# COPT-Public/LoRADS

Measured on AMD Instinct MI355X. Metric: ADMM iters/sec (+ inner CG-iters/sec), single-block n=20000 r=40, higher is better.
Workload: dtype f64

## Files before the change

### include/lorads_hip.h

```cpp
#ifndef LORADS_HIP_H
#define LORADS_HIP_H

#include <stdint.h>

#ifdef __cplusplus
extern "C" {
#endif

typedef struct lorads_hip_ctx lorads_hip_ctx;

typedef struct {
    int32_t n;
    int32_t rank;
    int32_t nrow;
    const int32_t *row_idx;
    const int32_t *a_ptr;
    const int32_t *a_row;
    const int32_t *a_col;
    const double *a_val;
    int32_t c_nnz;
    const int32_t *c_row;
    const int32_t *c_col;
    const double *c_val;
    int32_t is_lp;
// ... 59 lines not shown

int lorads_hip_triangle_cuts(lorads_hip_ctx *ctx, int32_t src, int32_t blk, double min_violation, int32_t max_cuts, int64_t *count,
                             int32_t *p, int32_t *q, int32_t *s, int8_t *cls, double *viol, int32_t *kept, int32_t *passes);

int lorads_hip_alm_to_admm(lorads_hip_ctx *ctx);
int lorads_hip_average_uv_to_v(lorads_hip_ctx *ctx);
int lorads_hip_scale_obj(lorads_hip_ctx *ctx, double s);
int lorads_hip_resize_rank(lorads_hip_ctx *ctx, const int32_t *new_rank);
int lorads_hip_set_mat(lorads_hip_ctx *ctx, int32_t which, int32_t blk, const double *colmajor);
int lorads_hip_get_mat(lorads_hip_ctx *ctx, int32_t which, int32_t blk, double *colmajor);
int lorads_hip_set_vec(lorads_hip_ctx *ctx, int32_t which, const double *v);
int lorads_hip_get_vec(lorads_hip_ctx *ctx, int32_t which, double *v);
int lorads_hip_set_allreduce(lorads_hip_ctx *ctx, lorads_hip_allreduce_fn fn, void *user);
void *lorads_hip_stream(lorads_hip_ctx *ctx);
int lorads_hip_set_allreduce_stream_ordered(lorads_hip_ctx *ctx, int32_t on);
int lorads_hip_set_separable(lorads_hip_ctx *ctx, int32_t on);
typedef int (*lorads_hip_scalar_exchange_fn)(void *user, double *vals, int32_t n);
int lorads_hip_set_scalar_exchange(lorads_hip_ctx *ctx, lorads_hip_scalar_exchange_fn fn, void *user);
int lorads_hip_selfcheck_allreduce(lorads_hip_ctx *ctx);

int lorads_hip_sync(lorads_hip_ctx *ctx);
int lorads_hip_spec_front_stats(lorads_hip_ctx *ctx, int64_t out[4]);

#ifdef __cplusplus
}
#endif
#endif
```

### lorads_amd/csrc/hip/graph.inc

```
struct MutSnap {
    InitArgs pend_init; Guard pend_init_g;
    Deferred pend_chk; Guard pend_chk_g;
    lorads_hip_ctx::PendDir pend_dir;
    lorads_hip_ctx::PendSegChk pend_segchk;
    bool pend_dual, pend_dual_virtual, virt_refresh, avg_folded, final_pending, stage_clean, merged_t_uv;
    EvalFinalArgs final_args;
    double *lambda, *lambda_alt;
    int ls_np, head;
    std::vector<unsigned char> blk;
    std::vector<const double *> wj_for;
};
struct GraphEntry {
    hipGraphExec_t exec = nullptr;
    MutSnap after;
    long d_matvec = 0;
    unsigned long long d_seq = 0;
};
struct GraphCache {
    std::map<std::vector<uint64_t>, GraphEntry> map;
    std::map<std::vector<uint64_t>, int> seen;
    long n_capture = 0, n_replay = 0;
};
void graph_cache_clear(lorads_hip_ctx *c) {
    if (!c->graphs) return;
    for (auto &kv : c->graphs->map)
        if (kv.second.exec) hipGraphExecDestroy(kv.second.exec);
    c->graphs->map.clear();
    c->graphs->seen.clear();
}
void graph_cache_free(lorads_hip_ctx *c) {
    graph_cache_clear(c);
    delete c->graphs;
    c->graphs = nullptr;
}
MutSnap snap_take(const lorads_hip_ctx *c) {
    MutSnap s;
    s.pend_init = c->pend_init; s.pend_init_g = c->pend_init_g; s.pend_chk = c->pend_chk; s.pend_chk_g = c->pend_chk_g;
    s.pend_dir = c->pend_dir; s.pend_segchk = c->pend_segchk;
    s.pend_dual = c->pend_dual; s.pend_dual_virtual = c->pend_dual_virtual; s.virt_refresh = c->virt_refresh; s.avg_folded = c->avg_folded;
// ... 62 lines not shown
int set_step_params(lorads_hip_ctx *c, double rho, double tol, int maxit) {
    const double v[4] = {rho, tol, c->pend_dual_rho, (double)maxit};
    const int mask = step_params_mask(c, v);
    if (!mask) return 0;
    hipLaunchKernelGGL(k_set_par, dim3(1), dim3(1), 0, c->stream, c->par, v[0], v[1], v[2], v[3], mask);
    for (int k = 0; k < 4; ++k)
        if ((mask >> k) & 1) { c->par_h[k] = v[k]; c->par_valid |= 1 << k; }
    return 0;
}

template <class F>
int graph_step(lorads_hip_ctx *c, std::vector<uint64_t> &key, F &&enqueue) {
    const MutSnap before = snap_take(c);
    if (!snap_quiet(before)) return enqueue();
    if (!c->graphs) c->graphs = new GraphCache();
    snap_key(c, before, key);
    auto it = c->graphs->map.find(key);
    if (it != c->graphs->map.end()) {
        const GraphEntry &e = it->second;
        HC(hipGraphLaunch(e.exec, c->stream));
        snap_put(c, e.after);
        c->n_matvec += e.d_matvec;
        c->pub_seq += e.d_seq;
        c->graphs->n_replay++;
        return 0;
    }
    if (c->graphs->seen.size() >= 4096) c->graphs->seen.clear();
    if (++c->graphs->seen[key] < 2) return enqueue();
    if (c->graphs->map.size() >= 256) graph_cache_clear(c);
    const long mv0 = c->n_matvec;
    const unsigned long long seq0 = c->pub_seq;
    auto give_up = [&](hipGraph_t g) {
        if (g) hipGraphDestroy(g);
        (void)hipGetLastError();
        c->opt_graph = false;
        snap_put(c, before);
        c->n_matvec = mv0;
        c->pub_seq = seq0;
        if (getenv("LORADS_HIP_VERBOSE")) fprintf(stderr, "lorads_hip: graph capture failed, launching step by step\n");
        return enqueue();
    };
    if (hipStreamBeginCapture(c->stream, hipStreamCaptureModeThreadLocal) != hipSuccess) return give_up(nullptr);
    const int rc = enqueue();
    hipGraph_t g = nullptr;
    const hipError_t e1 = hipStreamEndCapture(c->stream, &g);
    if (rc) {
        if (g) hipGraphDestroy(g);
        snap_put(c, before);
        c->n_matvec = mv0;
        c->pub_seq = seq0;
        return rc;
    }
    if (e1 != hipSuccess || !g) return give_up(g);
    GraphEntry ent;
    if (hipGraphInstantiate(&ent.exec, g, nullptr, nullptr, 0) != hipSuccess) return give_up(g);
    hipGraphDestroy(g);
    ent.after = snap_take(c);
    ent.d_matvec = c->n_matvec - mv0;
    ent.d_seq = c->pub_seq - seq0;
    HC(hipGraphLaunch(ent.exec, c->stream));
    c->graphs->map.emplace(key, std::move(ent));
    c->graphs->n_capture++;
    return 0;
}
```

### lorads_amd/csrc/hip/kernels.inc

```
template <int LG, bool V2, int NS>
struct Slice {
    static constexpr int W = V2 ? 2 : 1;
    __device__ static __forceinline__ void load(const double *__restrict__ row, int r, int lane, double (&v)[NS][W]) {
#pragma unroll
        for (int c = 0; c < NS; ++c) {
            const int j = (lane + c * LG) * W;
            const bool ok = j < r;
            const int jc = ok ? j : 0;
            if (V2) {
                const double2 t = *(const double2 *)(row + jc);
                v[c][0] = ok ? t.x : 0.0;
                v[c][W - 1] = ok ? t.y : 0.0;
            } else {
                const double t = row[jc];
                v[c][0] = ok ? t : 0.0;
            }
        }
    }
};

template <int LG, bool V2, int NS>
__device__ __forceinline__ double pair_dot(const double *__restrict__ X, const double *__restrict__ Y, int p, int q, int r,
                                           int lane) {
    constexpr int W = V2 ? 2 : 1;
// ... 97 lines not shown
                            : d.st ? !blocked_after(g, d, finish_deferred(d, dv, sh).done) : GATE_OPEN;
    if (live && act && lane64 == 0) {
        if (w_out) w_out[i] = s;
        if (vec) {
            const int gi = ra.b ? gi_pre : row_idx[i];
            if (mode == CV_SET) vec[gi] = s * scale;
            else if (mode == CV_ADD) vec[gi] += s * scale;
            else vec[gi] += s - cv[i];
        }
        if (cv) cv[i] = s;
    }
    if (ra.b) {
        double vd[2] = {0.0, 0.0};
        if (act && lane64 == 0) {
            const double bi = b_pre, t = bi - s * scale;
            vd[0] = t * t;
            vd[1] = bi * l_pre;
        }
        block_sum_n<2>(vd, sh);
        if (live && threadIdx.x == 0) { ra.part_v[blockIdx.x] = vd[0]; ra.part_d[blockIdx.x] = vd[1]; }
    }
}

template <int NS4, int NS>
__global__ __launch_bounds__(TPB) void k_eval_cw_obj(int nrow, int ell_w, const int *__restrict__ a_p, const double *__restrict__ a_val,
                                                     const int *__restrict__ a_q, const double *__restrict__ R, int r,
                                                     double *__restrict__ cv, const int *__restrict__ row_idx, double *__restrict__ vec,
                                                     ResArgs ra, int g_cw, int ne, const int *__restrict__ erow,
                                                     const int *__restrict__ ecol, const double *__restrict__ cval,
                                                     double *__restrict__ part_obj, Guard g, Deferred d) {
    __shared__ double sh[8];
    const Gate gt = gate_load(g);
    DefPriv dv{};
    if (d.st) dv = deferred_private(d);
    if ((int)blockIdx.x < g_cw) {
        constexpr int LG = 4, GR = 16;
        const int i = (blockIdx.x * TPB + threadIdx.x) >> 6, lane64 = threadIdx.x & 63;
        const int grp = lane64 / LG, lane = lane64 % LG;
        const bool act = i < nrow;
        const int ic = act ? i : 0;
        const int gi = row_idx[ic];
        const double bi = ra.b[gi], li = ra.lambda[gi];
        const int t0 = ic * ell_w, t1 = act ? t0 + ell_w : t0;
        double acc = 0.0;
        for (int t = t0 + grp; t < t1; t += GR) {
            const int p0 = a_p[t], q0 = a_q[t];
            const double c0 = a_val[t];
            acc += c0 * pair_dot<LG, true, NS4>(R, R, p0, q0, r, lane);
        }
        const double s = wave_sum(acc);
        const bool live = d.st ? !blocked_after(g, d, finish_deferred(d, dv, sh).done) : GATE_OPEN;
        if (live && act && lane64 == 0) { vec[gi] = s * 1.0; cv[i] = s; }
        double vd[2] = {0.0, 0.0};
        if (act && lane64 == 0) {
            const double t = bi - s * 1.0;
            vd[0] = t * t;
            vd[1] = bi * li;
        }
        block_sum_n<2>(vd, sh);
        if (live && threadIdx.x == 0) { ra.part_v[blockIdx.x] = vd[0]; ra.part_d[blockIdx.x] = vd[1]; }
        return;
    }
    constexpr int LG = 8, per = TPB / LG;
    const int bid = blockIdx.x - g_cw, nblk = gridDim.x - g_cw;
    const int lane = threadIdx.x % LG;
    double sacc = 0.0;
    for (int e = bid * per + threadIdx.x / LG; e < ne; e += nblk * per)
        sacc += pair_dot<LG, true, NS>(R, R, erow[e], ecol[e], r, lane) * cval[e];
    const bool live = d.st ? !blocked_after(g, d, finish_deferred(d, dv, sh).done) : GATE_OPEN;
    const double t = block_sum(sacc, sh);
    if (live && threadIdx.x == 0) part_obj[bid] = t;
}

__global__ void k_fill(size_t len, double v, double *__restrict__ y) {
    for (size_t i = (size_t)blockIdx.x * blockDim.x + threadIdx.x; i < len; i += (size_t)gridDim.x * blockDim.x) y[i] = v;
}

template <int LG, bool V2, int NS>
__device__ __forceinline__ void pair_dot_rd(const double *__restrict__ R, const double *__restrict__ D, int p, int q, int r,
                                            int lane, double &t1, double &t2) {
    constexpr int W = V2 ? 2 : 1;
    double rp[NS][W], rq[NS][W], dp[NS][W], dq[NS][W];
    Slice<LG, V2, NS>::load(R + (size_t)p * r, r, lane, rp);
    Slice<LG, V2, NS>::load(D + (size_t)q * r, r, lane, dq);
    Slice<LG, V2, NS>::load(R + (size_t)q * r, r, lane, rq);
    Slice<LG, V2, NS>::load(D + (size_t)p * r, r, lane, dp);
    double a1 = 0.0, a2 = 0.0, b1 = 0.0, b2 = 0.0;
#pragma unroll
    for (int c = 0; c < NS; ++c)
#pragma unroll
        for (int w = 0; w < W; ++w) {
            a1 += rp[c][w] * dq[c][w]; a2 += rq[c][w] * dp[c][w];
            b1 += dp[c][w] * dq[c][w]; b2 += dq[c][w] * dp[c][w];
        }
// ... 1761 lines not shown
    double acc = 0.0;
    for (int col = threadIdx.x; col < ncols; col += TPB) {
        double w = cobj[col];
        for (int t = ptr[col]; t < ptr[col + 1]; ++t) w += -lambda[grow[t]] * a[t];
        acc += fabs(w < 0.0 ? w : 0.0);
    }
    acc = block_sum(acc, sh);
    if (threadIdx.x == 0) *out = acc;
}

__global__ __launch_bounds__(TPB) void k_publish(const unsigned long long *__restrict__ src, int nwords, unsigned long long *dst,
                                                 unsigned long long *flag, unsigned long long *seq_dev) {
    const unsigned long long seq = *seq_dev + 1;
    for (int i = threadIdx.x; i < nwords; i += TPB) dst[i] = src[i];
    __threadfence_system();
    __syncthreads();
    if (threadIdx.x == 0) {
        *seq_dev = seq;
        __atomic_store_n(flag, seq, __ATOMIC_RELEASE);
        __threadfence_system();
    }
}

struct EvalFinalArgs {
    const double *part_v, *part_d, *obj_part;
    int np, nobj;
    double *out;
    Guard g;
};
__global__ __launch_bounds__(TPB) void k_publish_final(EvalFinalArgs fa, const unsigned long long *src, int nwords,
                                                       unsigned long long *dst, unsigned long long *flag, unsigned long long *seq_dev) {
    __shared__ double sh[12];
    const unsigned long long seq = *seq_dev + 1;
    constexpr int PW = 4;
    unsigned long long pre[PW];
#pragma unroll
    for (int k = 0; k < PW; ++k) {
        const int i = threadIdx.x + k * TPB;
        pre[k] = __builtin_nontemporal_load(src + (i < nwords ? i : 0));
    }
    const bool live = !blocked(fa.g);
    const double *const pp[3] = {fa.part_v, fa.part_d, fa.obj_part ? fa.obj_part : fa.part_v};
    const int nn[3] = {fa.np, fa.np, fa.obj_part ? fa.nobj : 0};
    double t3[3];
    private_partials_n<3>(pp, nn, t3);
    block_sum_n<3>(t3, sh);
    const double v = t3[0], d = t3[1], o = t3[2];
    if (live && threadIdx.x == 0) { fa.out[0] = v; fa.out[1] = d; if (fa.obj_part) fa.out[2] = o; }
    const bool own = (const double *)src == fa.out;
#pragma unroll
    for (int k = 0; k < PW; ++k) {
        const int i = threadIdx.x + k * TPB;
// ... 660 lines not shown
```

### lorads_amd/csrc/hip/lorads_hip.hip

```cpp
#include <hip/hip_runtime.h>

#include <fcntl.h>
#include <sys/file.h>
#include <unistd.h>

#include <algorithm>
#include <chrono>
#include <cmath>
#include <cstdint>
#include <cstdio>
#include <cstring>
#include <map>
#include <string>
#include <atomic>
#include <mutex>
#include <thread>
#include <tuple>
#include <type_traits>
#include <vector>

#include "lorads_hip.h"
#include "lorads_hip_dev.h"

namespace {
// ... 505 lines not shown
    long long n_dev_patterns = 0, n_checked_patterns = 0;
    bool opt_dense_cache = true;
    bool opt_front_diag = true;
    bool opt_eval_diag = true;
    bool opt_fold_avg = true;
    bool opt_tile_update = true;
    bool avg_folded = false;
    bool opt_front_lds = true;
    bool opt_front_cw = true;
    bool opt_fuse_cg0 = true;
    bool pend_dual_virtual = false;
    bool opt_spec_front = true;
    struct SpecFront {
        bool live = false;
        bool dual_seen = false;
        double rho = 0.0, rho_dual = 0.0;
        int wmode = 0;
        unsigned long long epoch = 0;
        CGState *reset = nullptr;
        int nreset = 0;
    } spec;
    unsigned long long spec_epoch = 0;
    long long n_spec_enq = 0, n_spec_adopt = 0, n_spec_discard = 0, n_spec_blocked = 0;
    bool opt_exact_refresh = false, opt_split_front = false;
    bool final_pending = false;
    EvalFinalArgs final_args;
    double *scal = nullptr;
    CGState *st = nullptr;
    CGState *st_shadow = nullptr;
    InitArgs pend_init{};
    Guard pend_init_g{};
    Deferred pend_chk{};
    Guard pend_chk_g{};
    bool opt_lazy_scalars = true;
    struct PendDir { int kind = 0; CGState *st = nullptr; double *r = nullptr, *p = nullptr; size_t len = 0; int gv = 0;
                     const double *rs_part = nullptr; int rs_np = 0; Guard g{}; bool seg = false; int half = 0;
                     const double *chk_part = nullptr; double chk_tol = 0; int chk_maxit = 0, chk_k = 0;
                     const double *rs_seg = nullptr; } pend_dir;
    struct PendSegChk { bool on = false; int half = 0, k = 0; const double *part = nullptr; double tol = 0; int maxit = 0;
                        bool ride_res = false; } pend_segchk;
    struct PendSegInit { bool on = false; int half = 0; double tol = 0; Guard front{}; const double *part_rr = nullptr, *part_b = nullptr; } pend_seginit;
    bool opt_seg_carry_init = true;
    lorads_hip_scalar_exchange_fn sx = nullptr;
    void *sx_user = nullptr;
    bool sx_pending = false;
    int sx_with_obj = 0;
// ... 81 lines not shown
        const size_t need = (std::max(rows_max, rows_all) + 3) / 4 + 1;
        if (need > ((size_t)1 << 27)) return fail_msg("cone dimension beyond 2^29 rows");
        c->maxpart = (int)std::max<size_t>((size_t)MINPART, (need + 255) & ~(size_t)255);
    }
    c->opt_pad_rank = env_on("LORADS_PAD_ODD_RANK");
    c->opt_dev_presolve = env_on("LORADS_DEV_PRESOLVE");
    c->opt_presolve_check = env_set("LORADS_PRESOLVE_CHECK");
    if (getenv("LORADS_DEV_PRESOLVE_MIN")) c->dev_presolve_min = (size_t)std::max(0ll, atoll(getenv("LORADS_DEV_PRESOLVE_MIN")));
    c->blk.resize(c->nb);
    for (int k = 0; k < c->nb; ++k)
        if (build_block(c, c->blk[k], prob->blocks[k])) return 1;
    if (build_merged(c, prob)) return 1;
    common_rank(c);
    refresh_merged(c);
    if (getenv("LORADS_HIP_VERBOSE"))
        fprintf(stderr, "lorads_hip: %d cone(s), merged view %s\n", c->nb, c->has_merged ? "on" : (c->merged_ok ? "off (ranks differ)" : "not applicable"));
    if (alloc_factors(c)) return 1;
    std::vector<double> hb(prob->b, prob->b + c->m);
    DevPool &M = c->mem;
    if (M.upload(&c->b, hb) || M.alloc(&c->lambda, (size_t)c->m) || M.alloc(&c->lambda_alt, (size_t)c->m) || M.alloc(&c->csum, (size_t)c->m + 2) ||
        M.alloc(&c->cstage, (size_t)c->m + 2 + MINPART) || M.alloc(&c->gram, 128) ||
        M.alloc(&c->q12, (size_t)2 * c->m + 2) || M.alloc(&c->part, (size_t)NSLOT * c->maxpart) ||
        M.alloc(&c->ctrl, 64 * sizeof(double) + sizeof(CGState) * (size_t)std::max(2 * c->nb, 1)) ||
        M.alloc(&c->ring_ab, (size_t)2 * c->L) || M.alloc(&c->par, 8) || M.alloc(&c->seq_dev, 2))
        return 1;
    HC(hipMemset(c->par, 0, sizeof(double) * 8));
    HC(hipMemset(c->seq_dev, 0, sizeof(unsigned long long) * 2));
    c->opt_graph = env_on("LORADS_GRAPH");
    c->opt_graph_batched = getenv("LORADS_GRAPH") && getenv("LORADS_GRAPH")[0] == '2';
    c->opt_graph_forced = getenv("LORADS_GRAPH") && (getenv("LORADS_GRAPH")[0] == '1' || getenv("LORADS_GRAPH")[0] == '2');
    if (M.alloc_pinned(&c->h_ctrl, 64 * sizeof(double) + sizeof(CGState) * (size_t)std::max(2 * c->nb, 1), hipHostMallocMapped) ||
        M.alloc_pinned(&c->h_flag, 64 / sizeof(*c->h_flag), hipHostMallocMapped))
        return 1;
    *c->h_flag = 0;
    HC(hipHostGetDevicePointer((void **)&c->h_ctrl_dev, c->h_ctrl, 0));
    HC(hipHostGetDevicePointer((void **)&c->h_flag_dev, c->h_flag, 0));
    c->use_publish = !getenv("LORADS_NO_PUBLISH");
    c->opt_lazy_scalars = env_on("LORADS_LAZY_SCALARS");
    c->opt_ar_fast = !env_set("LORADS_AR_PLAIN");
    c->opt_gram = env_on("LORADS_LBFGS_GRAM");
    c->opt_gram_single = getenv("LORADS_LBFGS_GRAM") && getenv("LORADS_LBFGS_GRAM")[0] == '2';
    c->opt_fuse_dir = env_on("LORADS_FUSE_DIR");
    c->opt_entry_bip = env_on("LORADS_ENTRY_BIP");
    c->opt_seg_carry = env_on("LORADS_SEG_CARRY");
    c->opt_seg_carry_init = env_on("LORADS_SEG_CARRY_INIT");
    c->opt_seg_virt = env_on("LORADS_SEG_VIRT");
    c->opt_seg_carry_dual = env_on("LORADS_SEG_CARRY_DUAL");
    c->opt_seg_carry_restart = env_on("LORADS_SEG_CARRY_RESTART");
    c->opt_cw_quad = env_on("LORADS_CW_QUAD");
    c->opt_front_cw = env_on("LORADS_FRONT_CW");
    c->opt_fuse_cg0 = env_on("LORADS_FUSE_CG0");
    c->opt_front_lds = env_on("LORADS_FRONT_LDS");
    c->opt_spec_front = env_on("LORADS_SPEC_FRONT");
    if (getenv("LORADS_SPEC_WINDOW")) c->spec_window = std::max(1, std::min(8, atoi(getenv("LORADS_SPEC_WINDOW"))));
    c->opt_fold_avg = env_on("LORADS_FOLD_AVG");
    c->opt_tile_update = env_on("LORADS_TILE_UPDATE");
    c->opt_eval_diag = env_on("LORADS_EVAL_DIAG");
    c->opt_front_diag = env_on("LORADS_FRONT_DIAG");
    c->opt_dense_cache = env_on("LORADS_DENSE_CACHE");
    c->opt_fuse_eval = env_on("LORADS_FUSE_EVAL");
    c->opt_dense_rem = env_on("LORADS_DENSE_REM");
    c->opt_exact_refresh = env_set("LORADS_EXACT_REFRESH");
    c->opt_split_front = env_set("LORADS_SPLIT_FRONT");
    c->scal = (double *)c->ctrl;
    c->st = (CGState *)(c->ctrl + 64 * sizeof(double));
    c->h_scal = (double *)c->h_ctrl;
    c->h_st = (CGState *)(c->h_ctrl + 64 * sizeof(double));
    HC(hipMemset(c->lambda, 0, sizeof(double) * (size_t)std::max(c->m, 1)));
    HC(hipMemset(c->csum, 0, sizeof(double) * (size_t)(c->m + 2)));
    HC(hipMemset(c->q12, 0, sizeof(double) * (size_t)(2 * c->m + 2)));
    HC(hipMemset(c->scal, 0, sizeof(double) * 64));
    HC(hipMemset(c->ring_ab, 0, sizeof(double) * (size_t)2 * c->L));
    HC(hipMemset(c->st, 0, sizeof(CGState) * (size_t)std::max(2 * c->nb, 1)));
    if (M.alloc(&c->st_shadow, (size_t)std::max(2 * c->nb, 1))) return 1;
    HC(hipMemset(c->st_shadow, 0, sizeof(CGState) * (size_t)std::max(2 * c->nb, 1)));
    c->persist = new PersistPlan();
// ... 860 lines not shown
    for (int i = 0; i < 16; ++i) ticks[i] = 0;
    if (c->persist && c->persist->valid && c->persist->stamps && c->persist_stamps) {
        HC(hipMemcpy(c->persist->h_stamps, c->persist->stamps, sizeof(unsigned long long) * 16, hipMemcpyDeviceToHost));
        for (int i = 0; i < 16; ++i) ticks[i] = c->persist->h_stamps[i];
        HC(hipMemset(c->persist->stamps, 0, sizeof(unsigned long long) * 16));
    }
    c->persist_stamps = enable != 0;
    return 0;
}

int lorads_hip_presolve_stats(lorads_hip_ctx *c, int64_t stats[2]) {
    spec_touch(c);
    stats[0] = c->n_dev_patterns;
    stats[1] = c->n_checked_patterns;
    return 0;
}

int lorads_hip_spec_front_stats(lorads_hip_ctx *c, int64_t out[4]) {
    if (!c || !out) return fail_msg("spec_front_stats: bad argument");
    out[0] = c->n_spec_enq; out[1] = c->n_spec_adopt; out[2] = c->n_spec_discard; out[3] = c->n_spec_blocked;
    return 0;
}

int lorads_hip_graph_stats(lorads_hip_ctx *c, int64_t stats[4]) {
    spec_touch(c);
    stats[0] = c->graphs ? c->graphs->n_capture : 0;
    stats[1] = c->graphs ? c->graphs->n_replay : 0;
    stats[2] = c->graphs ? (int64_t)c->graphs->map.size() : 0;
    stats[3] = graph_ok(c) ? 1 : 0;
    return 0;
}

int lorads_hip_algorithmic_bytes(lorads_hip_ctx *c, int32_t k, double *mv, double *cg) {
    spec_touch(c);
    if (k < 0 || k >= c->nb) return fail_msg("bad block");
    const Block &B = c->blk[k];
    const double F = 8.0 * (double)B.n * (double)B.rl;
    *mv = 4 * F + 32.0 * B.na + 16.0 * B.nrow;
    *cg = *mv + 9 * F;
    return 0;
}

}

#include "lanczos.inc"
#include "postsolve.inc"
// ... 6 lines not shown
```

### lorads_amd/csrc/hip/sweep.inc

```
void flush_pending(lorads_hip_ctx *c);
#define LAUNCH(kern, grid, ...)                                                                      \
    do {                                                                                             \
        const int grid__ = (int)(grid);                                                              \
        if (c->pend_init.st || c->pend_chk.st || c->pend_dir.kind || c->pend_dual || c->pend_dual_virtual || c->sep_pending || c->pend_seginit.on) flush_pending(c); \
        if (grid__ > 0) { ++c->n_launch; hipLaunchKernelGGL(kern, dim3(grid__), dim3(TPB), 0, c->stream, __VA_ARGS__); } \
    } while (0)
#define LAUNCH_LDS(kern, grid, lds, ...)                                                             \
    do {                                                                                             \
        const int grid__ = (int)(grid);                                                              \
        if (c->pend_init.st || c->pend_chk.st || c->pend_dir.kind || c->pend_dual || c->pend_dual_virtual || c->sep_pending || c->pend_seginit.on) flush_pending(c); \
        if (grid__ > 0) { ++c->n_launch; hipLaunchKernelGGL(kern, dim3(grid__), dim3(TPB), (size_t)(lds), c->stream, __VA_ARGS__); } \
    } while (0)
inline InitArgs take_init(lorads_hip_ctx *c) {
    const InitArgs ia = c->pend_init;
    c->pend_init = InitArgs{};
    return ia;
}
inline Deferred take_check(lorads_hip_ctx *c) {
    const Deferred d = c->pend_chk;
    c->pend_chk = Deferred{};
    return d;
}

struct Shape {
// ... 681 lines not shown
}
void refresh_after_solve(lorads_hip_ctx *c, Block &B, const int *need) {
    if (constr_by_recurrence(c, B) && B.t_uv_valid && B.nrow > 0) {
        const Deferred d = (c->pend_chk.st && need == &c->pend_chk.st->done && !c->pend_init.st) ? take_check(c) : Deferred{};
        LAUNCH(k_refresh_w, nblocks_for((size_t)B.nrow, TPB), B.nrow, (const double *)B.w_uv, B.cv, B.row_idx, c->csum,
               Guard{nullptr, need}, d, B.diag_only ? (const int *)B.diag_row : (const int *)nullptr,
               B.diag_only ? (const double *)B.diag_a : (const double *)nullptr);
        return;
    }
    constr_val(c, B, c->U + B.off, c->V + B.off, 1.0, B.cv, CV_DELTA, c->csum, Guard{nullptr, need});
}

void flush_final(lorads_hip_ctx *c);
int enqueue_publish(lorads_hip_ctx *c, size_t word0, size_t nwords) {
    if (c->sx_pending && (word0 > SX_WORD || word0 + nwords < SX_WORD + 4)) {
        const size_t w1 = std::max(word0 + nwords, (size_t)SX_WORD + 4);
        word0 = std::min(word0, (size_t)SX_WORD);
        nwords = w1 - word0;
    }
    const bool sep = c->sep_pending && !c->final_pending && c->sep_ex.n <= 4;
    if (sep) c->sep_pending = false;
    flush_pending(c);
    ++c->pub_seq;
    if (sep) {
        LAUNCH(k_publish_sep, 1, (const double *)c->sepbuf, c->scal, c->sep_with_obj, c->sep_ex.n, c->sep_ex.p[0], c->sep_ex.p[1], c->sep_ex.p[2],
               c->sep_ex.p[3], (const unsigned long long *)c->ctrl + word0, (int)nwords, (unsigned long long *)c->h_ctrl_dev + word0,
               c->h_flag_dev, c->seq_dev);
    } else if (c->final_pending) {
        LAUNCH(k_publish_final, 1, c->final_args, (const unsigned long long *)c->ctrl + word0, (int)nwords,
               (unsigned long long *)c->h_ctrl_dev + word0, c->h_flag_dev, c->seq_dev);
        c->final_pending = false;
    } else {
        LAUNCH(k_publish, 1, (const unsigned long long *)c->ctrl + word0, (int)nwords, (unsigned long long *)c->h_ctrl_dev + word0,
               c->h_flag_dev, c->seq_dev);
    }
    return 0;
}
int sx_exchange(lorads_hip_ctx *c) {
    if (!c->sx_pending) return 0;
    c->sx_pending = false;
    double v[4] = {c->h_scal[SX_WORD], c->h_scal[SX_WORD + 1], c->h_scal[SX_WORD + 2], c->h_scal[SX_WORD + 3]};
    if (!c->sx || c->sx(c->sx_user, v, 4)) return fail_msg("scalar exchange of separable shards failed (a rank that never arrived?)");
    c->n_sx++;
    c->h_scal[0] = v[0];
    c->h_scal[1] = v[1];
    if (c->sx_with_obj) c->h_scal[2] = v[2];
// ... 150 lines not shown
            }
        } else if (eval_follows && c->nb == 1 && stg == 0 && c->opt_lazy_scalars && constr_by_recurrence(c, B) && B.t_uv_valid &&
                   fused_front(c, B) && (B.use_cw || B.diag_only)) {
            c->virt_refresh = true;
        } else {
            if (stg == 2 * c->nb - 1 && (c->n_sweeps % 32) == 31) B.t_uv_valid = false;
            refresh_after_solve(c, B, &s.st->done);
        }
    }
}

int first_unfinished(lorads_hip_ctx *c, int first) {
    for (int stg = first; stg < 2 * c->nb; ++stg)
        if (c->h_st[stg].done == 0) return stg;
    return -1;
}

void flush_final(lorads_hip_ctx *c) {
    if (!c->final_pending) return;
    const EvalFinalArgs &fa = c->final_args;
    LAUNCH(k_eval_final, 1, fa.part_v, fa.part_d, fa.np, fa.out, fa.g, fa.obj_part, fa.nobj);
    c->final_pending = false;
}
int enqueue_eval(lorads_hip_ctx *c, int pair, const int *need, bool with_obj = true) {
    flush_final(c);
    const Guard g{nullptr, need};
    const bool vec = shard_vec(c);
    Block *Dc = solo(c);
    Block *D1 = (pair == LORADS_HIP_PAIR_UV && !vec && c->opt_eval_diag && Dc && Dc->diag_only && Dc->rc_w > 0 && Dc->nrow == c->m &&
                 c->m > 0 && Dc->w_uv && !c->avg_folded && !Dc->dense_c) ? Dc : nullptr;
    if (D1) {
    } else if (pair == LORADS_HIP_PAIR_UV && c->avg_folded && need) {
        c->avg_folded = false;
    } else if (pair == LORADS_HIP_PAIR_UV) {
        c->avg_folded = false;
        const Deferred d = (c->pend_chk.st && need == &c->pend_chk.st->done && !c->pend_init.st) ? take_check(c) : Deferred{};
        LAUNCH(k_average, grid1d(c->all_elem), c->all_elem, c->U, c->V, c->R, g, d);
    }
    Block *S1 = solo(c);
    if (S1 && (S1->nrow != c->m || S1->dense_c)) S1 = c->nb == 1 ? S1 : nullptr;
    const bool single = (S1 && S1->nrow == c->m) || (c->nb == 1 && c->blk[0].nrow == c->m);
    bool any_dense_a = false;
    for (auto &B0 : c->blk) any_dense_a = any_dense_a || B0.dense_a;
    const bool fold_res = single && !vec && c->m > 0 && !any_dense_a;
    c->ls_np = 0;
    double *dst = vec ? c->cstage : c->csum;
    std::vector<Block *> cones;
// ... 8 lines not shown
    }
    const bool ar_fast = vec && with_obj && c->ar_fast_all == 1 && cones.size() == 1;
    if ((!single || vec) && !(ar_fast && c->stage_clean)) LAUNCH(k_zero, grid1d((size_t)c->m), (size_t)c->m, dst, g);
    bool first_obj = true;
    const bool fold_obj = (c->nb == 1 || S1) && !vec;
    int nobj = 0, nres = 0;
    for (Block *bp : cones) {
        Block &B = *bp;
        if (D1 == &B && fold_res) {
            const Deferred d = (c->pend_chk.st && need == &c->pend_chk.st->done && !c->pend_init.st && !c->pend_dir.kind) ? take_check(c) : Deferred{};
            const Shape sh = shape_for(B.r);
            nres = nblocks_for((size_t)B.n, TPB / sh.lg);
            SHAPE_DISPATCH(sh, LAUNCH((k_eval_diag<LG_, V2_, NS_>), nres, B.n, (const double *)(c->U + B.off), (const double *)(c->V + B.off),
                                      c->R + B.off, B.r, B.rc_w, (const int *)B.rc_con, (const double *)B.diag_a,
                                      B.row_idx_identity ? (const int *)nullptr : (const int *)B.row_idx, B.cv, c->csum,
                                      (const double *)c->b, (const double *)c->lambda, part_slot(c, 8), part_slot(c, 9), g, d));
        } else if (fold_res && B.use_cw && with_obj && fold_obj && c->opt_fuse_eval && cw_quad(c, B) && B.nc > 0 && !B.dense_c &&
                   nblocks_for((size_t)B.nrow, TPB / 64) <= c->maxpart) {
            const Deferred d = (c->pend_chk.st && need == &c->pend_chk.st->done && !c->pend_init.st && !c->pend_dir.kind) ? take_check(c) : Deferred{};
            nres = nblocks_for((size_t)B.nrow, TPB / 64);
            nobj = std::min(nblocks_for((size_t)B.nc, TPB / 8), 2048);
            const int ns4 = (B.r + 7) / 8, ns = (B.r + 15) / 16;
            const ResArgs ra{c->b, c->lambda, part_slot(c, 8), part_slot(c, 9)};
#define EVF(A4, A8) LAUNCH((k_eval_cw_obj<A4, A8>), nres + nobj, B.nrow, B.ca_ell, (const int *)B.ca_row, (const double *)B.ca_val, (const int *)B.ca_col, \
                           (const double *)(c->R + B.off), B.r, B.cv, (const int *)B.row_idx, c->csum, ra, nres, B.nc, (const int *)B.c_row,           \
                           (const int *)B.c_col, (const double *)B.c_val, part_slot(c, 4), g, d)
            switch (ns4) {
            case 1: EVF(1, 1); break;
            case 2: EVF(2, 1); break;
            case 3: EVF(3, 2); break;
            case 4: EVF(4, 2); break;
            case 5: EVF(5, 3); break;
            default: EVF(6, 3); break;
            }
#undef EVF
            (void)ns;
            lp_col_values(c, B, c->R, c->R, g);
            continue;
        } else if (fold_res && B.use_cw && nblocks_for((size_t)B.nrow, TPB / 64) <= c->maxpart) {
            nres = cw(c, B, c->R + B.off, c->R + B.off, 1.0, (double *)nullptr, B.cv, (int)CV_SET, c->csum, g,
                      ResArgs{c->b, c->lambda, part_slot(c, 8), part_slot(c, 9)});
        } else if (fold_res) {
            pairdots(c, B.pa, c->R + B.off, c->R + B.off, B.r, B.T2, g);
            nres = std::min(nblocks_for((size_t)B.nrow, TPB / 8), 2048);
            LAUNCH(k_cv_res, nres, B.nrow, B.a_ptr, B.a_e, B.a_val, B.T2, B.cv, B.row_idx, c->csum, c->b, c->lambda, part_slot(c, 8),
                   part_slot(c, 9), g);
        } else {
            constr_val(c, B, c->R + B.off, c->R + B.off, 1.0, B.cv, (single && !vec) ? CV_SET : CV_ADD, dst, g);
        }
// ... 14 lines not shown
        nres = std::max(1, std::min(grid1d((size_t)c->m), 256));
        LAUNCH(k_commit_eval, nres, c->m, dst, c->csum, c->b, c->lambda, part_slot(c, 8), part_slot(c, 9), c->scal,
               ar_fast ? nobj : 0);
        c->stage_clean = ar_fast;
    } else if (!fold_res) {
        nres = std::min(grid1d((size_t)c->m), 1024);
        LAUNCH(k_eval_part, nres, c->m, c->b, c->csum, c->lambda, part_slot(c, 8), part_slot(c, 9), g);
    }
    const double *op = (fold_obj && nobj > 0) ? part_slot(c, 4) : (const double *)nullptr;
    if (c->ar && c->sep) {
        const SepExtra ex = c->sep_extra;
        c->sep_extra = SepExtra{};
        if (c->sx && ex.n == 0 && c->use_publish) {
            LAUNCH(k_sep_stage_local, 1, part_slot(c, 8), part_slot(c, 9), nres, op, nobj, (const double *)c->scal, g, with_obj ? 1 : 0, c->scal + SX_WORD);
            c->sx_pending = true; c->sx_with_obj = with_obj ? 1 : 0;
            return 0;
        }
        LAUNCH(k_sep_stage, 1, part_slot(c, 8), part_slot(c, 9), nres, op, nobj, (const double *)c->scal, g, with_obj ? 1 : 0, c->sepbuf, ex);
        flush_pending(c);
        if (allreduce_dev(c, c->sepbuf, 4 + ex.n)) return 1;
        c->sep_pending = true; c->sep_with_obj = with_obj ? 1 : 0; c->sep_ex = ex;
        return 0;
    }
    if (c->use_publish) {
        c->final_args = EvalFinalArgs{part_slot(c, 8), part_slot(c, 9), op, nres, nobj, c->scal, g};
        c->final_pending = true;
    } else {
        LAUNCH(k_eval_final, 1, part_slot(c, 8), part_slot(c, 9), nres, c->scal, g, op, nobj);
    }
    return 0;
}

int read_scalars_at(lorads_hip_ctx *c, const double *dptr, int count, double *out) {
    flush_pending(c);
    flush_final(c);
    if (c->launch_err) { const char *e = c->launch_err; c->launch_err = nullptr; hipStreamSynchronize(c->stream); return fail_msg(e); }
    HC(hipMemcpyAsync(c->h_scal + 32, dptr, sizeof(double) * (size_t)count, hipMemcpyDeviceToHost, c->stream));
    HC(hipStreamSynchronize(c->stream));
    memcpy(out, c->h_scal + 32, sizeof(double) * (size_t)count);
    return 0;
}
int read_scalars(lorads_hip_ctx *c, int first, int count, double *out) {
    if (publish_and_wait(c, (size_t)first, (size_t)count)) return 1;
    memcpy(out, c->h_scal + first, sizeof(double) * (size_t)count);
    return 0;
}

// ... 233 lines not shown
        if (read_states(c)) return 1;
    }
    return 0;
}

bool persist_ready(lorads_hip_ctx *c, int maxit);
int run_sweep_persist(lorads_hip_ctx *c, double rho, double tol, int maxit, bool with_eval);
int run_sweep(lorads_hip_ctx *c, double rho, double tol, int maxit, bool with_eval) {
    if (persist_ready(c, maxit)) { spec_touch(c); return run_sweep_persist(c, rho, tol, maxit, with_eval); }
    persist_touch(c);
    if (c->has_merged && !getenv("LORADS_NO_BATCH")) { spec_touch(c); return run_sweep_batched(c, rho, tol, maxit, with_eval); }
    int first = 0, resume = -1;
    bool first_pass = true, any_missed = false;
    const bool graph = graph_this_step(c, rho, tol, maxit);
    if (graph && set_step_params(c, rho, tol, maxit)) return 1;
    ParMode pm(c, graph);
    if (graph || maxit < 1) spec_touch(c);
    const bool spec = with_eval && !graph && spec_front_ok(c);
    for (;;) {
        const bool eval_now = with_eval && (!c->ar || first_pass);
        auto enq = [&]() -> int {
            if (first_pass && 2 * c->nb - 1 > TPB) HC(hipMemsetAsync(c->st, 0, sizeof(CGState) * (size_t)(2 * c->nb), c->stream));
            enqueue_sweep(c, first, resume, rho, tol, maxit, with_eval);
            if (eval_now && enqueue_eval(c, LORADS_HIP_PAIR_UV, c->nb ? &c->st[2 * c->nb - 1].done : nullptr)) return 1;
            return c->use_publish ? enqueue_publish(c, 0, state_words(c)) : 0;
        };
        if (graph && first_pass) {
            std::vector<uint64_t> key{1, (uint64_t)with_eval, (uint64_t)maxit, (uint64_t)((c->n_sweeps % 32) == 31)};
            if (graph_step(c, key, enq)) return 1;
        } else if (enq()) return 1;
        if (spec && first_pass) spec_front_enqueue(c, rho);
        if (c->use_publish ? wait_publish(c) : read_states(c)) return 1;
        if (eval_now && c->ar) any_missed = c->h_scal[5] > 0.5;
        const int stg = first_unfinished(c, first);
        if (first_pass && c->spec.live && stg >= 0) { c->spec.live = false; ++c->n_spec_blocked; }
        first_pass = false;
        if (stg < 0) break;
        first = stg;
        resume = c->h_st[stg].iter;
        c->n_resume++;
        c->merged.t_uv_valid = false;
        for (auto &B : c->blk) { B.t_uv_valid = false; B.w0_ready = false; B.wj_for = nullptr; }
    }
    if (with_eval && c->ar && any_missed) {
        if (enqueue_eval(c, LORADS_HIP_PAIR_UV, nullptr)) return 1;
        if (read_states(c)) return 1;
    }
    c->n_sweeps++;
// ... 4 lines not shown
```

### lorads_amd/host.py

```python
import ctypes as C
import os

import numpy as np

_HERE = os.path.dirname(os.path.abspath(__file__))
LIB_DIR = os.path.join(_HERE, "lib")
DEV_LIB = os.path.join(LIB_DIR, "liblorads_hip_dev.so")

PAIR_RR, PAIR_UV = 0, 1
MAT_R, MAT_U, MAT_V, MAT_GRAD = 0, 1, 2, 3
VEC_LAMBDA, VEC_CONSTR_SUM, VEC_Q1, VEC_Q2 = 0, 1, 2, 3

_dp = C.POINTER(C.c_double)
_ip = C.POINTER(C.c_int)
ALLREDUCE_FN = C.CFUNCTYPE(C.c_int, C.c_void_p, C.c_void_p, C.c_int, C.c_int)


class BackendStruct(C.Structure):
    _fields_ = [
        ("ctx", C.c_void_p),
        ("name", C.c_char_p),
        ("init_constr", C.CFUNCTYPE(C.c_int, C.c_void_p, C.c_int)),
        ("alm_cal_grad", C.CFUNCTYPE(C.c_int, C.c_void_p, C.c_double, _dp)),
        ("lbfgs_direction", C.CFUNCTYPE(C.c_int, C.c_void_p, C.c_int)),
# ... 485 lines not shown
        lib, ctx = self._hip()
        lib.lorads_hip_dual_infeasibility.argtypes = [C.c_void_p, C.c_double, C.c_int, C.c_int, _dp, _dp, _ip]
        nb = self.nblk
        v, lm, mv = C.c_double(), (C.c_double * max(nb, 1))(), C.c_int()
        _check(lib.lorads_hip_dual_infeasibility(ctx, tol, ncv, max_restarts, C.byref(v), lm, C.byref(mv)), "dual_infeasibility")
        return v.value, [lm[i] for i in range(nb)], mv.value

    def hip_block_image(self, blk=0):
        lib, ctx = self._hip()
        out = (C.c_int64 * 16)()
        lib.lorads_hip_block_image.argtypes = [C.c_void_p, C.c_int, C.POINTER(C.c_int64)]
        _check(lib.lorads_hip_block_image(ctx, blk, out), "block_image")
        keys = ["n", "rank", "nrow", "na", "nc", "pattern_a", "pattern_union", "dense_c", "dense_a", "diag_only", "entry_only", "use_cw",
                "has_gram", "front_cw", "slot_width", "bip_rows0"]
        return dict(zip(keys, [int(out[i]) for i in range(16)]))

    def hip_spec_front_stats(self):
        lib, ctx = self._hip()
        out = (C.c_int64 * 4)()
        lib.lorads_hip_spec_front_stats.argtypes = [C.c_void_p, C.POINTER(C.c_int64)]
        _check(lib.lorads_hip_spec_front_stats(ctx, out), "spec_front_stats")
        return dict(zip(["enqueued", "adopted", "discarded", "blocked"], [int(out[i]) for i in range(4)]))

    def hip_graph_stats(self):
        lib, ctx = self._hip()
        out = (C.c_int64 * 4)()
        lib.lorads_hip_graph_stats.argtypes = [C.c_void_p, C.POINTER(C.c_int64)]
        _check(lib.lorads_hip_graph_stats(ctx, out), "graph_stats")
        return dict(zip(["captured", "replayed", "held", "enabled"], [int(out[i]) for i in range(4)]))

    def hip_persist_stats(self):
        lib, ctx = self._hip()
        out = (C.c_int64 * 6)()
        lib.lorads_hip_persist_stats.argtypes = [C.c_void_p, C.POINTER(C.c_int64)]
        _check(lib.lorads_hip_persist_stats(ctx, out), "persist_stats")
        return dict(zip(["iterations", "available", "workgroups", "rows", "column_steps", "lds_bytes"], [int(out[i]) for i in range(6)]))

    def hip_persist_plan(self):
        lib, ctx = self._hip()
        out = (C.c_int64 * 8)()
        lib.lorads_hip_persist_plan.argtypes = [C.c_void_p, C.POINTER(C.c_int64)]
        _check(lib.lorads_hip_persist_plan(ctx, out), "persist_plan")
        return dict(zip(["tag", "xcd_map", "team", "sub_teams", "sub_team", "occ", "ncu", "allow_l2"], [int(out[i]) for i in range(8)]))

    def hip_persist_set_tag(self, tag):
        lib, ctx = self._hip()
# ... 365 lines not shown
```

Before: 9149.

## Fold eval reduction and host publish into the eval kernel's last-arriving block

Adds a two-level arrival counter (leaf and root) to k_eval_cw_obj. The last workgroup to finish reduces the residual and objective partials, writes the scalars and publishes the state words and sequence flag to host-visible memory. This replaces the separate k_eval_final and publish launches on eval steps for single-cone, non-allreduce runs. Partials are stored with agent-scope atomics so the closing block sees them coherently, at the cost of extra atomics and a serialized tail in the last block. Graph replay bookkeeping is extended to count folded and separate handovers.

Result: slower. 8712 (-4.8%).

```diff
diff --git a/include/lorads_hip.h b/include/lorads_hip.h
--- a/include/lorads_hip.h
+++ b/include/lorads_hip.h
@@ -105,6 +105,8 @@
 int lorads_hip_sync(lorads_hip_ctx *ctx);
 int lorads_hip_spec_front_stats(lorads_hip_ctx *ctx, int64_t out[4]);
 
+int lorads_hip_handover_stats(lorads_hip_ctx *ctx, int64_t out[2]);
+
 #ifdef __cplusplus
 }
 #endif
diff --git a/lorads_amd/csrc/hip/graph.inc b/lorads_amd/csrc/hip/graph.inc
--- a/lorads_amd/csrc/hip/graph.inc
+++ b/lorads_amd/csrc/hip/graph.inc
@@ -15,6 +15,7 @@
     MutSnap after;
     long d_matvec = 0;
     unsigned long long d_seq = 0;
+    long long d_folded = 0, d_separate = 0;
 };
 struct GraphCache {
     std::map<std::vector<uint64_t>, GraphEntry> map;
@@ -123,6 +124,8 @@
         snap_put(c, e.after);
         c->n_matvec += e.d_matvec;
         c->pub_seq += e.d_seq;
+        c->n_handover_folded += e.d_folded;
+        c->n_handover_separate += e.d_separate;
         c->graphs->n_replay++;
         return 0;
     }
@@ -131,6 +134,7 @@
     if (c->graphs->map.size() >= 256) graph_cache_clear(c);
     const long mv0 = c->n_matvec;
     const unsigned long long seq0 = c->pub_seq;
+    const long long fold0 = c->n_handover_folded, sep0 = c->n_handover_separate;
     auto give_up = [&](hipGraph_t g) {
         if (g) hipGraphDestroy(g);
         (void)hipGetLastError();
@@ -138,6 +142,7 @@
         snap_put(c, before);
         c->n_matvec = mv0;
         c->pub_seq = seq0;
+        c->n_handover_folded = fold0; c->n_handover_separate = sep0;
         if (getenv("LORADS_HIP_VERBOSE")) fprintf(stderr, "lorads_hip: graph capture failed, launching step by step\n");
         return enqueue();
     };
@@ -150,6 +155,7 @@
         snap_put(c, before);
         c->n_matvec = mv0;
         c->pub_seq = seq0;
+        c->n_handover_folded = fold0; c->n_handover_separate = sep0;
         return rc;
     }
     if (e1 != hipSuccess || !g) return give_up(g);
@@ -159,6 +165,8 @@
     ent.after = snap_take(c);
     ent.d_matvec = c->n_matvec - mv0;
     ent.d_seq = c->pub_seq - seq0;
+    ent.d_folded = c->n_handover_folded - fold0;
+    ent.d_separate = c->n_handover_separate - sep0;
     HC(hipGraphLaunch(ent.exec, c->stream));
     c->graphs->map.emplace(key, std::move(ent));
     c->graphs->n_capture++;
diff --git a/lorads_amd/csrc/hip/kernels.inc b/lorads_amd/csrc/hip/kernels.inc
--- a/lorads_amd/csrc/hip/kernels.inc
+++ b/lorads_amd/csrc/hip/kernels.inc
@@ -143,14 +143,112 @@
     }
 }
 
+struct EvalFinalArgs {
+    const double *part_v, *part_d, *obj_part;
+    int np, nobj;
+    double *out;
+    Guard g;
+};
+struct EvalClose {
+    unsigned long long *cnt;
+    int nleaf, leaf_base, leaf_rem;
+    EvalFinalArgs fa;
+    const unsigned long long *src;
+    int nwords;
+    unsigned long long *dst, *flag, *seq_dev;
+};
+__device__ __forceinline__ void store_partial(double *p, double v, bool through) {
+    if (through) __hip_atomic_store(p, v, __ATOMIC_RELAXED, __HIP_MEMORY_SCOPE_AGENT);
+    else *p = v;
+}
+template <int N>
+__device__ __forceinline__ void private_partials_n_coherent(const double *const (&part)[N], const int (&n)[N], double (&v)[N]) {
+    int nmax = 0;
+#pragma unroll
+    for (int a = 0; a < N; ++a) { v[a] = 0.0; nmax = n[a] > nmax ? n[a] : nmax; }
+    for (int i = threadIdx.x; i < nmax; i += 4 * TPB) {
+        double t[N][4];
+#pragma unroll
+        for (int a = 0; a < N; ++a)
+#pragma unroll
+            for (int k = 0; k < 4; ++k) {
+                const int j = i + k * TPB;
+                t[a][k] = __hip_atomic_load(part[a] + (j < n[a] ? j : 0), __ATOMIC_RELAXED, __HIP_MEMORY_SCOPE_AGENT);
+            }
+#pragma unroll
+        for (int a = 0; a < N; ++a)
+#pragma unroll
+            for (int k = 0; k < 4; ++k) v[a] += (i + k * TPB < n[a]) ? t[a][k] : 0.0;
+    }
+}
+__device__ __forceinline__ bool eval_arrive(const EvalClose &ec, bool wrote_state, int *last_sh) {
+    if (threadIdx.x == 0) {
+        if (wrote_state) __builtin_amdgcn_fence(__ATOMIC_RELEASE, "agent");
+        asm volatile("s_waitcnt vmcnt(0)" ::: "memory");
+        const int leaf = (int)(blockIdx.x % (unsigned)ec.nleaf);
+        const unsigned long long want = (unsigned long long)(ec.leaf_base + (leaf < ec.leaf_rem ? 1 : 0));
+        int last = 0;
+        if (__hip_atomic_fetch_add(ec.cnt + leaf, 1ull, __ATOMIC_RELAXED, __HIP_MEMORY_SCOPE_AGENT) + 1 == want)
+            last = __hip_atomic_fetch_add(ec.cnt + ec.nleaf, 1ull, __ATOMIC_RELAXED, __HIP_MEMORY_SCOPE_AGENT) + 1 == (unsigned long long)ec.nleaf;
+        *last_sh = last;
+    }
+    __syncthreads();
+    return *last_sh != 0;
+}
+__device__ __forceinline__ void eval_close(const EvalClose &ec, double *sh) {
+    const EvalFinalArgs &fa = ec.fa;
+    const unsigned long long seq = __hip_atomic_load(ec.seq_dev, __ATOMIC_RELAXED, __HIP_MEMORY_SCOPE_AGENT) + 1;
+    constexpr int PW = 4;
+    unsigned long long pre[PW];
+#pragma unroll
+    for (int k = 0; k < PW; ++k) {
+        const int i = threadIdx.x + k * TPB;
+        pre[k] = __hip_atomic_load(ec.src + (i < ec.nwords ? i : 0), __ATOMIC_RELAXED, __HIP_MEMORY_SCOPE_AGENT);
+    }
+    const int *ps = fa.g.skip ? fa.g.skip : &g_gate_words[0], *pn = fa.g.need ? fa.g.need : &g_gate_words[1];
+    Gate gt;
+    gt.vs = __hip_atomic_load(ps, __ATOMIC_RELAXED, __HIP_MEMORY_SCOPE_AGENT);
+    gt.vn = __hip_atomic_load(pn, __ATOMIC_RELAXED, __HIP_MEMORY_SCOPE_AGENT);
+    const bool live = !gate_blocked(fa.g, gt);
+    const double *const pp[3] = {fa.part_v, fa.part_d, fa.obj_part ? fa.obj_part : fa.part_v};
+    const int nn[3] = {fa.np, fa.np, fa.obj_part ? fa.nobj : 0};
+    double t3[3];
+    private_partials_n_coherent<3>(pp, nn, t3);
+    block_sum_n<3>(t3, sh);
+    const double v = t3[0], d = t3[1], o = t3[2];
+    if (live && threadIdx.x == 0) { fa.out[0] = v; fa.out[1] = d; if (fa.obj_part) fa.out[2] = o; }
+#pragma unroll
+    for (int k = 0; k < PW; ++k) {
+        const int i = threadIdx.x + k * TPB;
+        if (i >= ec.nwords) continue;
+        unsigned long long w = pre[k];
+        if (live) {
+            if (i == 0) w = (unsigned long long)__double_as_longlong(v);
+            else if (i == 1) w = (unsigned long long)__double_as_longlong(d);
+            else if (i == 2 && fa.obj_part) w = (unsigned long long)__double_as_longlong(o);
+        }
+        ec.dst[i] = w;
+    }
+    for (int i = threadIdx.x; i <= ec.nleaf; i += TPB) __hip_atomic_store(ec.cnt + i, 0ull, __ATOMIC_RELAXED, __HIP_MEMORY_SCOPE_AGENT);
+    __threadfence_system();
+    __syncthreads();
+    if (threadIdx.x == 0) {
+        *ec.seq_dev = seq;
+        __atomic_store_n(ec.flag, seq, __ATOMIC_RELEASE);
+        __threadfence_system();
+    }
+}
+
 template <int NS4, int NS>
 __global__ __launch_bounds__(TPB) void k_eval_cw_obj(int nrow, int ell_w, const int *__restrict__ a_p, const double *__restrict__ a_val,
                                                      const int *__restrict__ a_q, const double *__restrict__ R, int r,
                                                      double *__restrict__ cv, const int *__restrict__ row_idx, double *__restrict__ vec,
                                                      ResArgs ra, int g_cw, int ne, const int *__restrict__ erow,
                                                      const int *__restrict__ ecol, const double *__restrict__ cval,
-                                                     double *__restrict__ part_obj, Guard g, Deferred d) {
-    __shared__ double sh[8];
+                                                     double *__restrict__ part_obj, Guard g, Deferred d, EvalClose ec) {
+    __shared__ double sh[12];
+    __shared__ int last_sh;
+    const bool fold = ec.cnt != nullptr;
     const Gate gt = gate_load(g);
     DefPriv dv{};
     if (d.st) dv = deferred_private(d);
@@ -179,18 +277,20 @@
             vd[1] = bi * li;
         }
         block_sum_n<2>(vd, sh);
-        if (live && threadIdx.x == 0) { ra.part_v[blockIdx.x] = vd[0]; ra.part_d[blockIdx.x] = vd[1]; }
-        return;
-    }
-    constexpr int LG = 8, per = TPB / LG;
-    const int bid = blockIdx.x - g_cw, nblk = gridDim.x - g_cw;
-    const int lane = threadIdx.x % LG;
-    double sacc = 0.0;
-    for (int e = bid * per + threadIdx.x / LG; e < ne; e += nblk * per)
-        sacc += pair_dot<LG, true, NS>(R, R, erow[e], ecol[e], r, lane) * cval[e];
-    const bool live = d.st ? !blocked_after(g, d, finish_deferred(d, dv, sh).done) : GATE_OPEN;
-    const double t = block_sum(sacc, sh);
-    if (live && threadIdx.x == 0) part_obj[bid] = t;
+        if (live && threadIdx.x == 0) { store_partial(ra.part_v + blockIdx.x, vd[0], fold); store_partial(ra.part_d + blockIdx.x, vd[1], fold); }
+    } else {
+        constexpr int LG = 8, per = TPB / LG;
+        const int bid = blockIdx.x - g_cw, nblk = gridDim.x - g_cw;
+        const int lane = threadIdx.x % LG;
+        double sacc = 0.0;
+        for (int e = bid * per + threadIdx.x / LG; e < ne; e += nblk * per)
+            sacc += pair_dot<LG, true, NS>(R, R, erow[e], ecol[e], r, lane) * cval[e];
+        const bool live = d.st ? !blocked_after(g, d, finish_deferred(d, dv, sh).done) : GATE_OPEN;
+        const double t = block_sum(sacc, sh);
+        if (live && threadIdx.x == 0) store_partial(part_obj + bid, t, fold);
+    }
+    if (!fold) return;
+    if (eval_arrive(ec, blockIdx.x == 0 && d.st != nullptr, &last_sh)) eval_close(ec, sh);
 }
 
 __global__ void k_fill(size_t len, double v, double *__restrict__ y) {
@@ -1998,12 +2098,6 @@
     }
 }
 
-struct EvalFinalArgs {
-    const double *part_v, *part_d, *obj_part;
-    int np, nobj;
-    double *out;
-    Guard g;
-};
 __global__ __launch_bounds__(TPB) void k_publish_final(EvalFinalArgs fa, const unsigned long long *src, int nwords,
                                                        unsigned long long *dst, unsigned long long *flag, unsigned long long *seq_dev) {
     __shared__ double sh[12];
diff --git a/lorads_amd/csrc/hip/lorads_hip.hip b/lorads_amd/csrc/hip/lorads_hip.hip
--- a/lorads_amd/csrc/hip/lorads_hip.hip
+++ b/lorads_amd/csrc/hip/lorads_hip.hip
@@ -551,6 +551,10 @@
     } spec;
     unsigned long long spec_epoch = 0;
     long long n_spec_enq = 0, n_spec_adopt = 0, n_spec_discard = 0, n_spec_blocked = 0;
+    bool opt_fold_handover = true;
+    int handover_leaves = 64;
+    unsigned long long *eval_arrive = nullptr;
+    long long n_handover_folded = 0, n_handover_separate = 0;
     bool opt_exact_refresh = false, opt_split_front = false;
     bool final_pending = false;
     EvalFinalArgs final_args;
@@ -678,10 +682,11 @@
         M.alloc(&c->cstage, (size_t)c->m + 2 + MINPART) || M.alloc(&c->gram, 128) ||
         M.alloc(&c->q12, (size_t)2 * c->m + 2) || M.alloc(&c->part, (size_t)NSLOT * c->maxpart) ||
         M.alloc(&c->ctrl, 64 * sizeof(double) + sizeof(CGState) * (size_t)std::max(2 * c->nb, 1)) ||
-        M.alloc(&c->ring_ab, (size_t)2 * c->L) || M.alloc(&c->par, 8) || M.alloc(&c->seq_dev, 2))
+        M.alloc(&c->ring_ab, (size_t)2 * c->L) || M.alloc(&c->par, 8) || M.alloc(&c->seq_dev, 2) || M.alloc(&c->eval_arrive, 64 + 1))
         return 1;
     HC(hipMemset(c->par, 0, sizeof(double) * 8));
     HC(hipMemset(c->seq_dev, 0, sizeof(unsigned long long) * 2));
+    HC(hipMemset(c->eval_arrive, 0, sizeof(unsigned long long) * (64 + 1)));
     c->opt_graph = env_on("LORADS_GRAPH");
     c->opt_graph_batched = getenv("LORADS_GRAPH") && getenv("LORADS_GRAPH")[0] == '2';
     c->opt_graph_forced = getenv("LORADS_GRAPH") && (getenv("LORADS_GRAPH")[0] == '1' || getenv("LORADS_GRAPH")[0] == '2');
@@ -708,6 +713,8 @@
     c->opt_fuse_cg0 = env_on("LORADS_FUSE_CG0");
     c->opt_front_lds = env_on("LORADS_FRONT_LDS");
     c->opt_spec_front = env_on("LORADS_SPEC_FRONT");
+    c->opt_fold_handover = env_on("LORADS_FOLD_HANDOVER");
+    if (getenv("LORADS_HANDOVER_LEAVES")) c->handover_leaves = std::max(1, std::min(64, atoi(getenv("LORADS_HANDOVER_LEAVES"))));
     if (getenv("LORADS_SPEC_WINDOW")) c->spec_window = std::max(1, std::min(8, atoi(getenv("LORADS_SPEC_WINDOW"))));
     c->opt_fold_avg = env_on("LORADS_FOLD_AVG");
     c->opt_tile_update = env_on("LORADS_TILE_UPDATE");
@@ -1614,6 +1621,12 @@
     return 0;
 }
 
+int lorads_hip_handover_stats(lorads_hip_ctx *c, int64_t out[2]) {
+    if (!c || !out) return fail_msg("handover_stats: bad argument");
+    out[0] = c->n_handover_folded; out[1] = c->n_handover_separate;
+    return 0;
+}
+
 int lorads_hip_graph_stats(lorads_hip_ctx *c, int64_t stats[4]) {
     spec_touch(c);
     stats[0] = c->graphs ? c->graphs->n_capture : 0;
diff --git a/lorads_amd/csrc/hip/sweep.inc b/lorads_amd/csrc/hip/sweep.inc
--- a/lorads_amd/csrc/hip/sweep.inc
+++ b/lorads_amd/csrc/hip/sweep.inc
@@ -727,6 +727,7 @@
     if (sep) c->sep_pending = false;
     flush_pending(c);
     ++c->pub_seq;
+    ++c->n_handover_separate;
     if (sep) {
         LAUNCH(k_publish_sep, 1, (const double *)c->sepbuf, c->scal, c->sep_with_obj, c->sep_ex.n, c->sep_ex.p[0], c->sep_ex.p[1], c->sep_ex.p[2],
                c->sep_ex.p[3], (const unsigned long long *)c->ctrl + word0, (int)nwords, (unsigned long long *)c->h_ctrl_dev + word0,
@@ -923,7 +924,9 @@
     LAUNCH(k_eval_final, 1, fa.part_v, fa.part_d, fa.np, fa.out, fa.g, fa.obj_part, fa.nobj);
     c->final_pending = false;
 }
-int enqueue_eval(lorads_hip_ctx *c, int pair, const int *need, bool with_obj = true) {
+int enqueue_eval(lorads_hip_ctx *c, int pair, const int *need, bool with_obj = true, bool *handover = nullptr) {
+    const bool handover_follows = handover != nullptr;
+    bool folded = false;
     flush_final(c);
     const Guard g{nullptr, need};
     const bool vec = shard_vec(c);
@@ -978,9 +981,19 @@
             nobj = std::min(nblocks_for((size_t)B.nc, TPB / 8), 2048);
             const int ns4 = (B.r + 7) / 8, ns = (B.r + 15) / 16;
             const ResArgs ra{c->b, c->lambda, part_slot(c, 8), part_slot(c, 9)};
+            EvalClose ec{};
+            folded = handover_follows && c->opt_fold_handover && c->use_publish && !c->ar && !c->sx && !c->sx_pending && !c->sep_pending &&
+                     !B.is_lp && cones.size() == 1 && state_words(c) <= 4 * (size_t)TPB && (const double *)c->ctrl == c->scal;
+            if (folded) {
+                const int grid = nres + nobj, nleaf = std::min(c->handover_leaves, grid);
+                ec.cnt = c->eval_arrive; ec.nleaf = nleaf; ec.leaf_base = grid / nleaf; ec.leaf_rem = grid % nleaf;
+                ec.fa = EvalFinalArgs{part_slot(c, 8), part_slot(c, 9), part_slot(c, 4), nres, nobj, c->scal, g};
+                ec.src = (const unsigned long long *)c->ctrl; ec.nwords = (int)state_words(c);
+                ec.dst = (unsigned long long *)c->h_ctrl_dev; ec.flag = c->h_flag_dev; ec.seq_dev = c->seq_dev;
+            }
 #define EVF(A4, A8) LAUNCH((k_eval_cw_obj<A4, A8>), nres + nobj, B.nrow, B.ca_ell, (const int *)B.ca_row, (const double *)B.ca_val, (const int *)B.ca_col, \
                            (const double *)(c->R + B.off), B.r, B.cv, (const int *)B.row_idx, c->csum, ra, nres, B.nc, (const int *)B.c_row,           \
-                           (const int *)B.c_col, (const double *)B.c_val, part_slot(c, 4), g, d)
+                           (const int *)B.c_col, (const double *)B.c_val, part_slot(c, 4), g, d, ec)
             switch (ns4) {
             case 1: EVF(1, 1); break;
             case 2: EVF(2, 1); break;
@@ -1041,7 +1054,11 @@
         c->sep_pending = true; c->sep_with_obj = with_obj ? 1 : 0; c->sep_ex = ex;
         return 0;
     }
-    if (c->use_publish) {
+    if (folded) {
+        ++c->pub_seq;
+        ++c->n_handover_folded;
+        *handover = true;
+    } else if (c->use_publish) {
         c->final_args = EvalFinalArgs{part_slot(c, 8), part_slot(c, 9), op, nres, nobj, c->scal, g};
         c->final_pending = true;
     } else {
@@ -1321,8 +1338,9 @@
         auto enq = [&]() -> int {
             if (first_pass && 2 * c->nb - 1 > TPB) HC(hipMemsetAsync(c->st, 0, sizeof(CGState) * (size_t)(2 * c->nb), c->stream));
             enqueue_sweep(c, first, resume, rho, tol, maxit, with_eval);
-            if (eval_now && enqueue_eval(c, LORADS_HIP_PAIR_UV, c->nb ? &c->st[2 * c->nb - 1].done : nullptr)) return 1;
-            return c->use_publish ? enqueue_publish(c, 0, state_words(c)) : 0;
+            bool handed_over = false;
+            if (eval_now && enqueue_eval(c, LORADS_HIP_PAIR_UV, c->nb ? &c->st[2 * c->nb - 1].done : nullptr, true, &handed_over)) return 1;
+            return (c->use_publish && !handed_over) ? enqueue_publish(c, 0, state_words(c)) : 0;
         };
         if (graph && first_pass) {
             std::vector<uint64_t> key{1, (uint64_t)with_eval, (uint64_t)maxit, (uint64_t)((c->n_sweeps % 32) == 31)};
diff --git a/lorads_amd/host.py b/lorads_amd/host.py
--- a/lorads_amd/host.py
+++ b/lorads_amd/host.py
@@ -531,6 +531,13 @@
         _check(lib.lorads_hip_spec_front_stats(ctx, out), "spec_front_stats")
         return dict(zip(["enqueued", "adopted", "discarded", "blocked"], [int(out[i]) for i in range(4)]))
 
+    def hip_handover_stats(self):
+        lib, ctx = self._hip()
+        out = (C.c_int64 * 2)()
+        lib.lorads_hip_handover_stats.argtypes = [C.c_void_p, C.POINTER(C.c_int64)]
+        _check(lib.lorads_hip_handover_stats(ctx, out), "handover_stats")
+        return dict(zip(["folded", "separate"], [int(out[i]) for i in range(2)]))
+
     def hip_graph_stats(self):
         lib, ctx = self._hip()
         out = (C.c_int64 * 4)()
```
